# ChainSafe/Spectre

Hardware: AMD Instinct MI355X
Metric: BN254 G1 MSM n=2^20 throughput (higher is better)
Workload: dtype u256; 1 GPU; msm_g1_2pow20; n=1048576, seed=42, parallelism=shard1:window, pipeline_depth=3, scalars=canonical

## Files before the change

spectre_amd/csrc/ff.hpp:

```cpp
#pragma once
#include <stdint.h>
#include <string.h>

#if defined(__HIPCC__) || defined(__HIP_DEVICE_COMPILE__)
#include <hip/hip_runtime.h>
#define FF_HD __host__ __device__ __forceinline__
#else
#define FF_HD inline
#endif

struct fp256 {
    uint32_t l[8];
};

struct FqP {
    static constexpr bool kAsmMul = true;
    static constexpr bool kChainAddSub = true;
    FF_HD static constexpr uint32_t mod(int i) {
        constexpr uint32_t M[8] = {0xd87cfd47u, 0x3c208c16u, 0x6871ca8du, 0x97816a91u,
                                   0x8181585du, 0xb85045b6u, 0xe131a029u, 0x30644e72u};
        return M[i];
    }
    FF_HD static constexpr uint32_t inv() { return 0xe4866389u; }
    FF_HD static constexpr uint32_t r2(int i) {
// ... 61 lines not shown
        o.l[i] = (uint32_t)d;
        brw = (d >> 32) & 1;
    }
    return (uint32_t)brw;
}
FF_HD uint32_t ff_add_raw(fp256& o, const fp256& a, const fp256& b) {
    uint64_t c = 0;
    for (int i = 0; i < 8; i++) {
        c += (uint64_t)a.l[i] + b.l[i];
        o.l[i] = (uint32_t)c;
        c >>= 32;
    }
    return (uint32_t)c;
}
FF_HD uint32_t ff_adc_(uint32_t a, uint32_t b, uint32_t& carry) {
#if defined(__has_builtin) && __has_builtin(__builtin_addc)
    unsigned out;
    const uint32_t r = __builtin_addc(a, b, carry, &out);
    carry = out;
    return r;
#else
    const uint64_t s = (uint64_t)a + b + carry;
    carry = (uint32_t)(s >> 32);
    return (uint32_t)s;
#endif
}
FF_HD uint32_t ff_sbb_(uint32_t a, uint32_t b, uint32_t& borrow) {
#if defined(__has_builtin) && __has_builtin(__builtin_subc)
    unsigned out;
    const uint32_t r = __builtin_subc(a, b, borrow, &out);
    borrow = out;
    return r;
#else
    const uint64_t d = (uint64_t)a - b - borrow;
    borrow = (uint32_t)(d >> 32) & 1;
    return (uint32_t)d;
#endif
}
template <class C> FF_HD void ff_cond_sub_mod_chain_(fp256& o, uint32_t extra) {
    uint32_t d[8], brw = 0;
    for (int i = 0; i < 8; i++) d[i] = ff_sbb_(o.l[i], C::mod(i), brw);
    const bool keep = extra != 0 || brw == 0;
    for (int i = 0; i < 8; i++) o.l[i] = keep ? d[i] : o.l[i];
}
template <class C> FF_HD void ff_cond_sub_mod(fp256& o, uint32_t extra) {
    if constexpr (C::kChainAddSub) {
        ff_cond_sub_mod_chain_<C>(o, extra);
    } else if (extra || ff_geq_mod<C>(o)) {
        uint64_t brw = 0;
        for (int i = 0; i < 8; i++) {
            uint64_t d = (uint64_t)o.l[i] - C::mod(i) - brw;
            o.l[i] = (uint32_t)d;
            brw = (d >> 32) & 1;
        }
    }
}
template <class C> FF_HD void ff_add(fp256& o, const fp256& a, const fp256& b) {
    if constexpr (C::kChainAddSub) {
        uint32_t c = 0;
        for (int i = 0; i < 8; i++) o.l[i] = ff_adc_(a.l[i], b.l[i], c);
        ff_cond_sub_mod_chain_<C>(o, c);
    } else {
        uint32_t c = ff_add_raw(o, a, b);
        ff_cond_sub_mod<C>(o, c);
    }
}
template <class C> FF_HD void ff_sub(fp256& o, const fp256& a, const fp256& b) {
    if constexpr (C::kChainAddSub) {
        uint32_t brw = 0;
        for (int i = 0; i < 8; i++) o.l[i] = ff_sbb_(a.l[i], b.l[i], brw);
        const uint32_t mask = 0u - brw;
        uint32_t c = 0;
        for (int i = 0; i < 8; i++) o.l[i] = ff_adc_(o.l[i], C::mod(i) & mask, c);
    } else if (ff_sub_raw(o, a, b)) {
        uint64_t c = 0;
        for (int i = 0; i < 8; i++) {
            c += (uint64_t)o.l[i] + C::mod(i);
            o.l[i] = (uint32_t)c;
            c >>= 32;
        }
    }
}
template <class C> FF_HD void ff_neg(fp256& o, const fp256& a) {
    if (ff_is_zero(a)) { o = a; return; }
    fp256 m;
    for (int i = 0; i < 8; i++) m.l[i] = C::mod(i);
    ff_sub_raw(o, m, a);
}

template <class C> FF_HD void ff_mul_cios(fp256& o, const fp256& a, const fp256& b) {
    uint32_t t[10];
    for (int i = 0; i < 10; i++) t[i] = 0;
    for (int i = 0; i < 8; i++) {
        uint64_t cc = 0;
        const uint32_t ai = a.l[i];
        for (int j = 0; j < 8; j++) {
            uint64_t x = (uint64_t)ai * b.l[j] + t[j] + (uint32_t)cc;
            t[j] = (uint32_t)x;
            cc = x >> 32;
        }
        uint64_t x = (uint64_t)t[8] + (uint32_t)cc;
        t[8] = (uint32_t)x;
        t[9] = (uint32_t)(x >> 32);
        const uint32_t m = t[0] * C::inv();
        uint64_t x2 = (uint64_t)m * C::mod(0) + t[0];
        cc = x2 >> 32;
        for (int j = 1; j < 8; j++) {
            x2 = (uint64_t)m * C::mod(j) + t[j] + (uint32_t)cc;
            t[j - 1] = (uint32_t)x2;
            cc = x2 >> 32;
        }
        x2 = (uint64_t)t[8] + (uint32_t)cc;
        t[7] = (uint32_t)x2;
        t[8] = t[9] + (uint32_t)(x2 >> 32);
    }
    for (int i = 0; i < 8; i++) o.l[i] = t[i];
    ff_cond_sub_mod<C>(o, t[8]);
}
#if defined(__HIP_DEVICE_COMPILE__) && !defined(SPECTRE_NO_ASM_MUL)
#define FF_HAVE_ASM_MUL 1
#endif

#if defined(FF_HAVE_ASM_MUL)
__device__ __forceinline__ void ff_mad64_(uint64_t& acc, uint32_t& ovf,
                                          uint32_t a, uint32_t b) {
    uint64_t c;
    asm volatile("v_mad_u64_u32 %0, %2, %3, %4, %0\n\t"
                 "v_addc_co_u32 %1, %2, 0, %1, %2"
                 : "+v"(acc), "+v"(ovf), "=s"(c)
                 : "v"(a), "v"(b));
}
__device__ __forceinline__ void ff_mad64_s_(uint64_t& acc, uint32_t& ovf,
                                            uint32_t a, uint32_t b_uniform) {
    uint64_t c;
    asm volatile("v_mad_u64_u32 %0, %2, %3, %4, %0\n\t"
                 "v_addc_co_u32 %1, %2, 0, %1, %2"
                 : "+v"(acc), "+v"(ovf), "=s"(c)
                 : "v"(a), "s"(b_uniform));
}
template <class C, int K>
__device__ __forceinline__ void detail_ff_low_cols(uint64_t& acc,
                                                   uint32_t& ovf,
                                                   const uint32_t* a,
                                                   const uint32_t* b,
                                                   uint32_t* m) {
    if constexpr (K < 8) {
#pragma unroll
        for (int i = 0; i <= K; i++) ff_mad64_(acc, ovf, a[i], b[K - i]);
#pragma unroll
        for (int i = 0; i < K; i++) ff_mad64_s_(acc, ovf, m[i], C::mod(K - i));
        m[K] = (uint32_t)acc * C::inv();
        ff_mad64_s_(acc, ovf, m[K], C::mod(0));
        acc = (acc >> 32) | ((uint64_t)ovf << 32);
        ovf = 0;
        detail_ff_low_cols<C, K + 1>(acc, ovf, a, b, m);
    }
}
template <class C, int K>
__device__ __forceinline__ void detail_ff_high_cols(uint64_t& acc,
                                                    uint32_t& ovf,
                                                    const uint32_t* a,
                                                    const uint32_t* b,
                                                    const uint32_t* m,
                                                    uint32_t* out) {
    if constexpr (K < 15) {
#pragma unroll
// ... 6 lines not shown
        detail_ff_high_cols<C, K + 1>(acc, ovf, a, b, m, out);
    }
}
template <class C>
__device__ __forceinline__ void ff_mul_cols(fp256& o, const fp256& A,
                                            const fp256& B) {
    uint32_t m[8];
    uint64_t acc = 0;
    uint32_t ovf = 0;
    detail_ff_low_cols<C, 0>(acc, ovf, A.l, B.l, m);
    detail_ff_high_cols<C, 8>(acc, ovf, A.l, B.l, m, o.l);
    o.l[7] = (uint32_t)acc;
    ff_cond_sub_mod<C>(o, (uint32_t)(acc >> 32));
}

template <int K>
__device__ __forceinline__ void detail_ff_sqr_col(uint64_t& acc, uint32_t& ovf,
                                                  const uint32_t* a,
                                                  const uint32_t* adj,
                                                  const uint32_t* dbl) {
#pragma unroll
    for (int i = K < 8 ? 0 : K - 7; 2 * i + 1 < K; i++)
        ff_mad64_(acc, ovf, a[i], dbl[K - i]);
    if constexpr (K % 2) ff_mad64_(acc, ovf, a[K / 2], adj[K / 2 + 1]);
    else ff_mad64_(acc, ovf, a[K / 2], a[K / 2]);
}
template <class C, int K>
__device__ __forceinline__ void detail_ff_sqr_low_cols(uint64_t& acc,
                                                       uint32_t& ovf,
                                                       const uint32_t* a,
                                                       const uint32_t* adj,
                                                       const uint32_t* dbl,
                                                       uint32_t* m) {
    if constexpr (K < 8) {
        detail_ff_sqr_col<K>(acc, ovf, a, adj, dbl);
#pragma unroll
        for (int i = 0; i < K; i++) ff_mad64_s_(acc, ovf, m[i], C::mod(K - i));
        m[K] = (uint32_t)acc * C::inv();
        ff_mad64_s_(acc, ovf, m[K], C::mod(0));
        acc = (acc >> 32) | ((uint64_t)ovf << 32);
        ovf = 0;
        detail_ff_sqr_low_cols<C, K + 1>(acc, ovf, a, adj, dbl, m);
    }
}
template <class C, int K>
__device__ __forceinline__ void detail_ff_sqr_high_cols(uint64_t& acc,
                                                        uint32_t& ovf,
                                                        const uint32_t* a,
                                                        const uint32_t* adj,
                                                        const uint32_t* dbl,
                                                        const uint32_t* m,
                                                        uint32_t* out) {
    if constexpr (K < 15) {
        detail_ff_sqr_col<K>(acc, ovf, a, adj, dbl);
#pragma unroll
        for (int i = K - 7; i < 8; i++) ff_mad64_s_(acc, ovf, m[i], C::mod(K - i));
        out[K - 8] = (uint32_t)acc;
        acc = (acc >> 32) | ((uint64_t)ovf << 32);
        ovf = 0;
        detail_ff_sqr_high_cols<C, K + 1>(acc, ovf, a, adj, dbl, m, out);
    }
}
template <class C>
__device__ __forceinline__ void ff_sqr_cols(fp256& o, const fp256& A) {
    static_assert(C::mod(7) < 0x80000000u,
                  "the doubled limbs drop bit 255: reduced elements must be "
                  "below 2^255");
    uint32_t a[8], adj[8], dbl[8], m[8];
#pragma unroll
    for (int i = 0; i < 8; i++) a[i] = A.l[i];
    adj[0] = dbl[0] = 0;
#pragma unroll
    for (int j = 1; j < 8; j++) {
        adj[j] = a[j] << 1;
        dbl[j] = (a[j] << 1) | (a[j - 1] >> 31);
    }
    uint64_t acc = 0;
    uint32_t ovf = 0;
    detail_ff_sqr_low_cols<C, 0>(acc, ovf, a, adj, dbl, m);
    detail_ff_sqr_high_cols<C, 8>(acc, ovf, a, adj, dbl, m, o.l);
    o.l[7] = (uint32_t)acc;
    ff_cond_sub_mod<C>(o, (uint32_t)(acc >> 32));
}
#endif

template <class C> FF_HD void ff_mul(fp256& o, const fp256& a, const fp256& b) {
#if defined(FF_HAVE_ASM_MUL)
    if constexpr (C::kAsmMul) {
        ff_mul_cols<C>(o, a, b);
        return;
    }
#endif
    ff_mul_cios<C>(o, a, b);
}

template <class C> FF_HD void ff_sqr(fp256& o, const fp256& a) {
#if defined(FF_HAVE_ASM_MUL)
    if constexpr (C::kAsmMul) {
        ff_sqr_cols<C>(o, a);
        return;
    }
#endif
    ff_mul<C>(o, a, a);
}

template <class C> FF_HD void ff_to_mont(fp256& o, const fp256& a_canon) {
    fp256 r2;
    for (int i = 0; i < 8; i++) r2.l[i] = C::r2(i);
    ff_mul<C>(o, a_canon, r2);
}
template <class C> FF_HD void ff_from_mont(fp256& o, const fp256& a) {
    fp256 one;
    ff_set_zero(one);
    one.l[0] = 1;
    ff_mul<C>(o, a, one);
}

template <class C> FF_HD void ff_pow_u32(fp256& o, const fp256& a, uint32_t e) {
    fp256 acc, base = a;
    ff_set_one<C>(acc);
    while (e) {
        if (e & 1) ff_mul<C>(acc, acc, base);
        e >>= 1;
        if (e) ff_sqr<C>(base, base);
    }
    o = acc;
}
template <class C> FF_HD void ff_inv(fp256& o, const fp256& a) {
    static_assert(C::mod(0) >= 2u, "m - 2 must not borrow out of the low word");
    fp256 acc, base = a;
    ff_set_one<C>(acc);
#pragma unroll 1
    for (uint32_t w = 0; w < 8; w++) {
        uint32_t bits = C::mod(0) - 2u;
#pragma unroll
        for (uint32_t i = 1; i < 8; i++) bits = w == i ? C::mod(i) : bits;
#pragma unroll 1
        for (uint32_t b = 0; b < 32; b++) {
            if ((bits >> b) & 1) ff_mul<C>(acc, acc, base);
            ff_sqr<C>(base, base);
        }
    }
    o = acc;
}

FF_HD void ff_from_bytes(fp256& o, const uint8_t* b) { memcpy(o.l, b, 32); }
FF_HD void ff_to_bytes(uint8_t* b, const fp256& a) { memcpy(b, a.l, 32); }

using Fq = FqP;
using Fr = FrP;

#if defined(__HIPCC__) || defined(__HIP_DEVICE_COMPILE__)
__device__ __forceinline__ void lds_split_ld(const uint4* lds4, uint32_t lo,
                                             uint32_t dist, fp256& o) {
    uint4 l = lds4[lo], h = lds4[dist + lo];
    memcpy(&o.l[0], &l, 16);
    memcpy(&o.l[4], &h, 16);
}
__device__ __forceinline__ void lds_split_st(uint4* lds4, uint32_t lo,
                                             uint32_t dist, const fp256& v) {
    uint4 l, h;
    memcpy(&l, &v.l[0], 16);
    memcpy(&h, &v.l[4], 16);
    lds4[lo] = l;
    lds4[dist + lo] = h;
}
#endif
```

spectre_amd/csrc/g1.hpp:

```cpp
#pragma once
#include "ff.hpp"

struct g1_affine {
    fp256 x, y;
};
struct g1_jac {
    fp256 X, Y, Z;
};

FF_HD bool g1a_is_inf(const g1_affine& p) { return ff_is_zero(p.x) && ff_is_zero(p.y); }
FF_HD void g1j_set_inf(g1_jac& p) {
    ff_set_one<Fq>(p.X);
    ff_set_one<Fq>(p.Y);
    ff_set_zero(p.Z);
}
FF_HD bool g1j_is_inf(const g1_jac& p) { return ff_is_zero(p.Z); }
FF_HD void g1j_from_affine(g1_jac& o, const g1_affine& p) {
    if (g1a_is_inf(p)) { g1j_set_inf(o); return; }
    o.X = p.x;
    o.Y = p.y;
    ff_set_one<Fq>(o.Z);
}

FF_HD void g1j_dbl_ip(g1_jac& p) {
    if (g1j_is_inf(p)) return;
    fp256 A, B, C, D, E, F;
    ff_sqr<Fq>(A, p.X);
    ff_sqr<Fq>(B, p.Y);
    ff_sqr<Fq>(C, B);
    ff_add<Fq>(D, p.X, B);
    ff_sqr<Fq>(D, D);
    ff_sub<Fq>(D, D, A);
    ff_sub<Fq>(D, D, C);
    ff_add<Fq>(D, D, D);
    ff_add<Fq>(E, A, A);
    ff_add<Fq>(E, E, A);
    ff_sqr<Fq>(F, E);
    ff_mul<Fq>(p.Z, p.Y, p.Z);
    ff_add<Fq>(p.Z, p.Z, p.Z);
    ff_sub<Fq>(p.X, F, D);
    ff_sub<Fq>(p.X, p.X, D);
    ff_sub<Fq>(D, D, p.X);
    ff_mul<Fq>(D, E, D);
    ff_add<Fq>(C, C, C);
    ff_add<Fq>(C, C, C);
    ff_add<Fq>(C, C, C);
    ff_sub<Fq>(p.Y, D, C);
}

FF_HD void g1j_madd_ip(g1_jac& p, const g1_affine& q) {
    if (g1a_is_inf(q)) return;
    if (g1j_is_inf(p)) { g1j_from_affine(p, q); return; }
    fp256 Z1Z1, U2, S2, H, HH, I, J, rr, V;
    ff_sqr<Fq>(Z1Z1, p.Z);
    ff_mul<Fq>(U2, q.x, Z1Z1);
    ff_mul<Fq>(S2, q.y, p.Z);
    ff_mul<Fq>(S2, S2, Z1Z1);
    ff_sub<Fq>(H, U2, p.X);
    ff_sub<Fq>(rr, S2, p.Y);
    if (ff_is_zero(H)) {
        if (ff_is_zero(rr)) { g1j_dbl_ip(p); return; }
        g1j_set_inf(p);
        return;
    }
    ff_add<Fq>(rr, rr, rr);
    ff_sqr<Fq>(HH, H);
    ff_add<Fq>(I, HH, HH);
    ff_add<Fq>(I, I, I);
    ff_mul<Fq>(J, H, I);
    ff_mul<Fq>(V, p.X, I);
    ff_add<Fq>(p.Z, p.Z, H);
    ff_sqr<Fq>(p.Z, p.Z);
    ff_sub<Fq>(p.Z, p.Z, Z1Z1);
    ff_sub<Fq>(p.Z, p.Z, HH);
    ff_sqr<Fq>(H, rr);
    ff_sub<Fq>(H, H, J);
    ff_sub<Fq>(H, H, V);
    ff_sub<Fq>(H, H, V);
    ff_sub<Fq>(V, V, H);
    ff_mul<Fq>(V, rr, V);
    ff_mul<Fq>(J, p.Y, J);
    ff_add<Fq>(J, J, J);
    ff_sub<Fq>(p.Y, V, J);
    p.X = H;
}

FF_HD void g1j_add_ip(g1_jac& p, const g1_jac& q) {
    if (g1j_is_inf(q)) return;
    if (g1j_is_inf(p)) { p = q; return; }
    fp256 Z1Z1, Z2Z2, U1, U2, S1, S2, H, I, J, rr, V;
    ff_sqr<Fq>(Z1Z1, p.Z);
    ff_sqr<Fq>(Z2Z2, q.Z);
    ff_mul<Fq>(U1, p.X, Z2Z2);
    ff_mul<Fq>(U2, q.X, Z1Z1);
    ff_mul<Fq>(S1, p.Y, q.Z);
    ff_mul<Fq>(S1, S1, Z2Z2);
    ff_mul<Fq>(S2, q.Y, p.Z);
    ff_mul<Fq>(S2, S2, Z1Z1);
    ff_sub<Fq>(H, U2, U1);
    ff_sub<Fq>(rr, S2, S1);
    if (ff_is_zero(H)) {
        if (ff_is_zero(rr)) { g1j_dbl_ip(p); return; }
        g1j_set_inf(p);
        return;
    }
    ff_add<Fq>(rr, rr, rr);
    ff_add<Fq>(I, H, H);
    ff_sqr<Fq>(I, I);
    ff_mul<Fq>(J, H, I);
    ff_mul<Fq>(V, U1, I);
    ff_add<Fq>(p.Z, p.Z, q.Z);
    ff_sqr<Fq>(p.Z, p.Z);
    ff_sub<Fq>(p.Z, p.Z, Z1Z1);
    ff_sub<Fq>(p.Z, p.Z, Z2Z2);
    ff_mul<Fq>(p.Z, p.Z, H);
    ff_sqr<Fq>(H, rr);
    ff_sub<Fq>(H, H, J);
    ff_sub<Fq>(H, H, V);
    ff_sub<Fq>(H, H, V);
    ff_sub<Fq>(V, V, H);
    ff_mul<Fq>(V, rr, V);
    ff_mul<Fq>(J, S1, J);
    ff_add<Fq>(J, J, J);
    ff_sub<Fq>(p.Y, V, J);
    p.X = H;
}


FF_HD void g1j_to_affine(g1_affine& o, const g1_jac& p) {
    if (g1j_is_inf(p)) {
        ff_set_zero(o.x);
        ff_set_zero(o.y);
        return;
    }
    fp256 zi, zi2, zi3;
    ff_inv<Fq>(zi, p.Z);
    ff_sqr<Fq>(zi2, zi);
    ff_mul<Fq>(zi3, zi2, zi);
    ff_mul<Fq>(o.x, p.X, zi2);
    ff_mul<Fq>(o.y, p.Y, zi3);
}
```

spectre_amd/csrc/internal.hpp:

```cpp
#pragma once
#include <hip/hip_runtime.h>
#include "spectre_gpu.h"
#include "ff.hpp"
#include "g1.hpp"
#include "powtab.hpp"
#include <array>
#include <map>
#include <mutex>
#include <string>
#include <vector>

#define MSM_WBITS 16
#define MSM_NWIN 16
#define MSM_BPW (1u << (MSM_WBITS - 1))
#ifndef MSM_CHUNK
#define MSM_CHUNK SPECTRE_MSM_TAIL_CHUNK
#endif
#define MSM_CPW (MSM_BPW / MSM_CHUNK)
#define MSM_LO SPECTRE_MSM_TAIL_LO
#define MSM_HI (MSM_CPW / MSM_LO)
static_assert(MSM_CPW % MSM_LO == 0, "chunks per window: a multiple of MSM_LO");
static_assert((MSM_CHUNK & (MSM_CHUNK - 1)) == 0 && (MSM_LO & (MSM_LO - 1)) == 0,
              "the host fold multiplies by doubling");
#define MSM_ACC_E_MIN 8
#define MSM_ACC_E_MAX 64
#define MSM_ACC_TARGET_BLOCKS 2

void set_err(const char* fmt, ...);

#define HIP_TRY(x)                                                        \
    do {                                                                  \
        hipError_t _e = (x);                                              \
        if (_e != hipSuccess) {                                           \
            set_err("%s:%d %s: %s", __FILE__, __LINE__, #x,               \
                    hipGetErrorString(_e));                               \
            return -2;                                                    \
        }                                                                 \
    } while (0)

#define RC_TRY(x)                                                         \
    do {                                                                  \
        int _rc = (x);                                                    \
        if (_rc) return _rc;                                              \
    } while (0)

template <typename T, bool kPinned = false>
struct DevBuf {
    T* ptr = nullptr;
    size_t cap = 0;
    int reserve(size_t n) {
        if (cap >= n) return 0;
        release();
        void* p = nullptr;
        if (kPinned) HIP_TRY(hipHostMalloc(&p, n * sizeof(T)));
        else HIP_TRY(hipMalloc(&p, n * sizeof(T)));
        ptr = (T*)p;
        cap = n;
        return 0;
    }
    void release() {
        if (ptr) (void)(kPinned ? hipHostFree(ptr) : hipFree(ptr));
        ptr = nullptr;
        cap = 0;
    }
};
template <typename T>
using PinnedBuf = DevBuf<T, true>;
template <typename... B>
void release_all(B&... b) {
    (b.release(), ...);
}

struct NttPlan {
    uint32_t npass = 0;
    uint32_t k[3] = {};
    DevBuf<fp256> tw[3];
    DevBuf<fp256> twB;
    PowTable omega = {};
    void release() { release_all(tw[0], tw[1], tw[2], twB); }
};

#define MSM_SLOTS 3
struct MsmSlot {
    hipStream_t stream = nullptr;
    DevBuf<uint32_t> d_keys_in, d_keys_out, d_vals_in, d_vals_out;
    DevBuf<uint8_t> d_sort_tmp;
    DevBuf<uint32_t> d_firstK, d_lastK;
    DevBuf<g1_jac> d_firstP, d_lastP;
    DevBuf<uint32_t> d_offsets;
    DevBuf<g1_jac> d_buckets;
    DevBuf<g1_jac> d_red;
    PinnedBuf<g1_jac> h_wins;
    g1_jac* pending_dst = nullptr;
    uint32_t pending_n = 0;
    void release(hipStream_t shared) {
        release_all(d_keys_in, d_keys_out, d_vals_in, d_vals_out, d_sort_tmp,
                    d_firstK, d_lastK, d_firstP, d_lastP, d_offsets,
                    d_buckets, d_red, h_wins);
        if (stream && stream != shared) (void)hipStreamDestroy(stream);
        stream = nullptr;
    }
};

struct DeviceState {
    int device_id = 0;
    hipStream_t stream = nullptr;
    MsmSlot slots[MSM_SLOTS];
    int next_slot = 0;
    int num_cus = 0;
    int acc_resident_blocks = 0;
    DevBuf<uint8_t> d_scalars;
    DevBuf<g1_affine> d_bases;
    std::map<std::array<uint64_t, 3>, DevBuf<g1_affine>> bases_cache;
    DevBuf<fp256> d_ntt_io;
    PinnedBuf<uint8_t> h_stage[2];
    hipEvent_t stage_ev[2] = {nullptr, nullptr};
    DevBuf<uint8_t> d_call;
    PinnedBuf<uint8_t> h_call;
    std::map<std::array<uint8_t, 40>, NttPlan> plans;
    void release() {
        for (auto& sl : slots) sl.release(stream);
        release_all(d_scalars, d_bases, d_ntt_io, h_stage[0], h_stage[1],
                    d_call, h_call);
        for (auto& kv : bases_cache) kv.second.release();
        bases_cache.clear();
        for (auto& kv : plans) kv.second.release();
        plans.clear();
        for (auto& e : stage_ev) {
            if (e) (void)hipEventDestroy(e);
            e = nullptr;
        }
        if (stream) (void)hipStreamDestroy(stream);
        stream = nullptr;
    }
};

#define CALL_PINNED_BYTES \
    (SPECTRE_OPEN_MAX_POLYS * SPECTRE_POLY_EVAL_MAX_POINTS * 32u)
inline int call_finish(DeviceState& ds, void* dst = nullptr,
                       const void* d_src = nullptr, size_t bytes = 0) {
    if (dst) {
        RC_TRY(ds.h_call.reserve(CALL_PINNED_BYTES));
        HIP_TRY(hipMemcpyAsync(ds.h_call.ptr, d_src, bytes,
                               hipMemcpyDeviceToHost, ds.stream));
    }
    HIP_TRY(hipStreamSynchronize(ds.stream));
    HIP_TRY(hipGetLastError());
    if (dst) memcpy(dst, ds.h_call.ptr, bytes);
    return 0;
}

struct spectre_gpu_ctx {
    std::vector<DeviceState> devs;
    std::recursive_mutex mu;
    uint32_t msm_acc_entries = 0;
    uint32_t fr_scan_tile = 0;
    bool ntt_force3 = false;
};

struct MsmCall {
    const g1_affine* d_bases;
    const uint8_t* d_scalars;
    uint32_t nbatch;
    uint64_t n;
    uint32_t flags;
    uint32_t w_lo, w_cnt;
};

int msm_device(spectre_gpu_ctx* ctx, int dev, const MsmCall& call,
               g1_jac* winsums_host, double* stage_ms, bool sync, int slot);

uint32_t msm_acc_auto_entries(uint64_t entries, uint32_t cus,
                              uint32_t resident_blocks);

int msm_slot_drain(spectre_gpu_ctx* ctx, int dev, int slot);

void msm_fold_window(const g1_jac& p0, const g1_jac& p1, const g1_jac& p2,
                     g1_jac& out);

int fr_gate_eval_device(spectre_gpu_ctx* ctx, int dev,
                        const fp256* const* cols, uint32_t ncols,
// ... 56 lines not shown
```

spectre_amd/csrc/msm.hip:

```cpp
#include "internal.hpp"
#include <hipcub/hipcub.hpp>

#define THREADS 256
#define PT_KERNEL __global__ __launch_bounds__(THREADS, 2)
#ifndef MSM_ACC_THREADS
#define MSM_ACC_THREADS 256
#endif
#define ACC_KERNEL __global__ __launch_bounds__(MSM_ACC_THREADS, 2)

__global__ void k_msm_digits(const uint8_t* __restrict__ scalars, uint64_t n,
                             uint32_t nbatch, int canonical, uint32_t w_lo,
                             uint32_t w_cnt,
                             uint32_t* __restrict__ keys,
                             uint32_t* __restrict__ vals) {
    uint64_t i = (uint64_t)blockIdx.x * blockDim.x + threadIdx.x;
    if (i >= n) return;
    const uint32_t nb_local = w_cnt * MSM_BPW;
    const uint32_t skip_key = nbatch * nb_local;
    for (uint32_t b = 0; b < nbatch; b++) {
        fp256 s;
        ff_from_bytes(s, scalars + 32 * (b * n + i));
        if (!canonical) ff_from_mont<Fr>(s, s);
        uint32_t carry = 0;
        for (int w = 0; w < MSM_NWIN; w++) {
            const uint32_t bit0 = (uint32_t)w * MSM_WBITS;
            const uint32_t li = bit0 >> 5, sh = bit0 & 31;
            uint64_t pair = (uint64_t)s.l[li];
            if (li < 7) pair |= (uint64_t)s.l[li + 1] << 32;
            uint32_t d =
                ((uint32_t)(pair >> sh) & ((1u << MSM_WBITS) - 1)) + carry;
            const uint32_t half = 1u << (MSM_WBITS - 1);
            const uint32_t full = 1u << MSM_WBITS;
            uint32_t key, val = (uint32_t)i;
            if (d == 0) {
                carry = 0;
                key = skip_key;
            } else if (d <= half) {
                carry = 0;
                key = b * nb_local + ((uint32_t)w - w_lo) * MSM_BPW + (d - 1);
            } else if (d == full) {
                carry = 1;
                key = skip_key;
            } else {
                carry = 1;
                key = b * nb_local + ((uint32_t)w - w_lo) * MSM_BPW +
                      (full - d - 1);
                val |= 0x80000000u;
            }
            if ((uint32_t)w < w_lo || (uint32_t)w >= w_lo + w_cnt) continue;
            const uint64_t slot =
                ((uint64_t)b * w_cnt + ((uint32_t)w - w_lo)) * n + i;
            keys[slot] = key;
            vals[slot] = val;
        }
    }
}

__global__ void k_bucket_offsets(const uint32_t* __restrict__ keys,
                                 uint64_t nent, uint32_t nb_total,
                                 uint32_t* __restrict__ off) {
    uint32_t b = blockIdx.x * blockDim.x + threadIdx.x;
    if (b > nb_total) return;
    uint64_t lo = 0, hi = nent;
    while (lo < hi) {
        uint64_t mid = (lo + hi) >> 1;
        if (keys[mid] < b) lo = mid + 1;
        else hi = mid;
    }
    off[b] = (uint32_t)lo;
}

#define ACC_WAVES (MSM_ACC_THREADS / 64)
__device__ __forceinline__ void glds16(const void* src, uint4* wave_dst) {
    __builtin_amdgcn_global_load_lds(
        (const __attribute__((address_space(1))) void*)src,
        (__attribute__((address_space(3))) void*)wave_dst, 16, 0, 0);
}
__device__ __forceinline__ void glds_landed() {
    asm volatile("s_waitcnt vmcnt(0)" ::: "memory");
}
__device__ __forceinline__ void lds_reads_done() {
    asm volatile("s_waitcnt lgkmcnt(0)" ::: "memory");
}

ACC_KERNEL void k_bucket_acc(const uint32_t* __restrict__ off,
                            const uint32_t* __restrict__ keys,
                            const uint32_t* __restrict__ vals,
                            const g1_affine* __restrict__ bases,
                            uint32_t nb_total, uint32_t E,
                            g1_jac* __restrict__ buckets,
                            uint32_t* __restrict__ firstK,
                            g1_jac* __restrict__ firstP,
                            uint32_t* __restrict__ lastK,
                            g1_jac* __restrict__ lastP) {
    __shared__ uint4 stage[ACC_WAVES][8][64];
    const uint32_t ent = off[nb_total];
    const uint32_t t = blockIdx.x * blockDim.x + threadIdx.x;
    const uint64_t lo = (uint64_t)t * E;
    if (lo >= ent) return;
    const uint32_t cnt = ent - lo < E ? (uint32_t)(ent - lo) : E;
    const uint4* kq = (const uint4*)(keys + lo);
    const uint4* vq = (const uint4*)(vals + lo);
    const uint32_t lane = threadIdx.x & 63;
    uint4(*st)[64] = stage[threadIdx.x >> 6];
    glds16(kq, st[4]);
    glds16(vq, st[6]);
    glds_landed();
    uint32_t k = st[4][lane].x;
    {
        const uint4* src = (const uint4*)(bases + (st[6][lane].x & 0x7fffffffu));
        for (int c = 0; c < 4; c++) glds16(src + c, st[c]);
    }
    g1_jac acc;
    g1j_set_inf(acc);
    bool first = true;
    for (uint32_t i = 0; i < cnt; i++) {
        glds_landed();
        const uint32_t q = 4 + ((i >> 2) & 1);
        const uint32_t kj = ((const uint32_t*)&st[q][lane])[i & 3];
        const uint32_t v = ((const uint32_t*)&st[q + 2][lane])[i & 3];
        g1_affine p;
        {
            const uint4 x0 = st[0][lane], x1 = st[1][lane];
            const uint4 y0 = st[2][lane], y1 = st[3][lane];
            p.x.l[0] = x0.x; p.x.l[1] = x0.y; p.x.l[2] = x0.z; p.x.l[3] = x0.w;
            p.x.l[4] = x1.x; p.x.l[5] = x1.y; p.x.l[6] = x1.z; p.x.l[7] = x1.w;
            p.y.l[0] = y0.x; p.y.l[1] = y0.y; p.y.l[2] = y0.z; p.y.l[3] = y0.w;
            p.y.l[4] = y1.x; p.y.l[5] = y1.y; p.y.l[6] = y1.z; p.y.l[7] = y1.w;
        }
        if (i + 1 < cnt) {
            const uint32_t qn = 6 + (((i + 1) >> 2) & 1);
            const uint32_t vn = ((const uint32_t*)&st[qn][lane])[(i + 1) & 3];
            lds_reads_done();
            if ((i & 3) == 0 && i + 4 < cnt) {
                const uint32_t qf = 4 + (((i >> 2) + 1) & 1);
                glds16(kq + (i >> 2) + 1, st[qf]);
                glds16(vq + (i >> 2) + 1, st[qf + 2]);
            }
            const uint4* src = (const uint4*)(bases + (vn & 0x7fffffffu));
            for (int c = 0; c < 4; c++) glds16(src + c, st[c]);
        }
        if (kj != k) {
            if (first) {
                firstK[t] = k;
                firstP[t] = acc;
                first = false;
            } else {
                buckets[k] = acc;
            }
            g1j_set_inf(acc);
            k = kj;
        }
        if (v & 0x80000000u) ff_neg<Fq>(p.y, p.y);
        g1j_madd_ip(acc, p);
    }
    if (first) {
        firstK[t] = k;
        firstP[t] = acc;
        lastK[t] = 0xffffffffu;
    } else {
        lastK[t] = k;
        lastP[t] = acc;
    }
}

ACC_KERNEL void k_bucket_fix(const uint32_t* __restrict__ off,
                            const uint32_t* __restrict__ firstK,
                            const g1_jac* __restrict__ firstP,
                            const uint32_t* __restrict__ lastK,
                            const g1_jac* __restrict__ lastP,
                            uint32_t nb_total, uint32_t E,
                            g1_jac* __restrict__ buckets) {
    uint32_t b = blockIdx.x * blockDim.x + threadIdx.x;
    if (b >= nb_total) return;
    uint32_t s = off[b], e = off[b + 1];
    if (s == e) {
        g1j_set_inf(buckets[b]);
        return;
    }
    uint32_t ts = s / E, te = (e - 1) / E;
    const uint32_t ent = off[nb_total];
    if (ts == te && (s % E) && (e % E) && e != ent)
        return;
    g1_jac acc;
    g1j_set_inf(acc);
    for (uint32_t t = ts; t <= te; t++) {
        if (firstK[t] == b) g1j_add_ip(acc, firstP[t]);
        if (lastK[t] == b) g1j_add_ip(acc, lastP[t]);
    }
    buckets[b] = acc;
}

PT_KERNEL void k_window_chunks(const g1_jac* __restrict__ buckets,
                               uint32_t total_chunks,
                               g1_jac* __restrict__ outW,
                               g1_jac* __restrict__ outT) {
    uint32_t t = blockIdx.x * blockDim.x + threadIdx.x;
    if (t >= total_chunks) return;
    const g1_jac* B = buckets + (uint64_t)t * MSM_CHUNK;
    g1_jac accT, accW;
    g1j_set_inf(accT);
    g1j_set_inf(accW);
    for (int j = MSM_CHUNK - 1; j >= 0; j--) {
        g1j_add_ip(accT, B[j]);
        g1j_add_ip(accW, accT);
    }
    outW[t] = accW;
    outT[t] = accT;
}

#ifndef WSUM_THREADS
#define WSUM_THREADS 512
#endif
static_assert(MSM_CPW % WSUM_THREADS == 0, "role 0 shares");
static_assert(WSUM_THREADS % MSM_LO == 0 && MSM_HI % (WSUM_THREADS / MSM_LO) == 0,
              "column shares");
static_assert(MSM_HI <= WSUM_THREADS && WSUM_THREADS % MSM_HI == 0 &&
              MSM_LO % (WSUM_THREADS / MSM_HI) == 0, "row shares");
__global__ __launch_bounds__(WSUM_THREADS, 2) void k_window_tail(
    const g1_jac* __restrict__ inW, const g1_jac* __restrict__ inT,
    g1_jac* __restrict__ out) {
    __shared__ g1_jac lds[WSUM_THREADS / 2];
    const uint32_t w = blockIdx.x / 3, role = blockIdx.x % 3;
    const uint32_t t = threadIdx.x;
    const uint32_t M = role == 0 ? 0 : role == 1 ? MSM_LO : MSM_HI;
    const g1_jac* src;
    uint32_t stride, cnt;
    if (role == 0) {
        src = inW + (uint64_t)w * MSM_CPW + t;
        stride = WSUM_THREADS;
        cnt = MSM_CPW / WSUM_THREADS;
    } else if (role == 1) {
        cnt = MSM_HI / (WSUM_THREADS / MSM_LO);
        src = inT + (uint64_t)w * MSM_CPW + (t / MSM_LO) * cnt * MSM_LO +
              t % MSM_LO;
        stride = MSM_LO;
    } else {
        cnt = MSM_LO / (WSUM_THREADS / MSM_HI);
        src = inT + (uint64_t)w * MSM_CPW + (t % MSM_HI) * MSM_LO +
              (t / MSM_HI) * cnt;
        stride = 1;
    }
    g1_jac acc;
    g1j_set_inf(acc);
    for (uint32_t j = 0; j < cnt; j++) g1j_add_ip(acc, src[(uint64_t)j * stride]);
    for (uint32_t k = WSUM_THREADS / 2; k >= 1; k >>= 1) {
        if (2 * k == M && t < M) {
            if (t == 0) g1j_set_inf(acc);
            if (!g1j_is_inf(acc)) {
                g1_jac r;
                g1j_set_inf(r);
                for (uint32_t bit = M >> 1; bit; bit >>= 1) {
                    g1j_dbl_ip(r);
                    if (t & bit) g1j_add_ip(r, acc);
                }
                acc = r;
            }
        }
        if (t >= k && t < 2 * k) lds[t - k] = acc;
        __syncthreads();
        if (t < k) g1j_add_ip(acc, lds[t]);
        __syncthreads();
    }
    if (t == 0) out[blockIdx.x] = acc;
}

uint32_t msm_acc_auto_entries(uint64_t entries, uint32_t cus,
                              uint32_t resident_blocks) {
    uint32_t per_cu = resident_blocks ? resident_blocks : 1;
    if (per_cu > MSM_ACC_TARGET_BLOCKS) per_cu = MSM_ACC_TARGET_BLOCKS;
    const uint64_t threads =
        (uint64_t)(cus ? cus : 1) * per_cu * MSM_ACC_THREADS;
    if (entries >= threads * MSM_ACC_E_MAX) return MSM_ACC_E_MAX;
    uint64_t e = (entries + threads - 1) / threads;
    e = (e + 3) & ~3ull;
    if (e < MSM_ACC_E_MIN) e = MSM_ACC_E_MIN;
    if (e > MSM_ACC_E_MAX) e = MSM_ACC_E_MAX;
    return (uint32_t)e;
}

static int ensure_acc_geometry(DeviceState& dstate) {
    if (dstate.acc_resident_blocks) return 0;
    int cus = 0, nb = 0;
    HIP_TRY(hipDeviceGetAttribute(&cus, hipDeviceAttributeMultiprocessorCount,
                                  dstate.device_id));
    HIP_TRY(hipOccupancyMaxActiveBlocksPerMultiprocessor(
        &nb, k_bucket_acc, MSM_ACC_THREADS, 0));
    dstate.num_cus = cus > 0 ? cus : 1;
    dstate.acc_resident_blocks = nb > 0 ? nb : 1;
    return 0;
}

static int ensure_msm_scratch(MsmSlot& ds, uint64_t ent, uint32_t nwin,
                              uint32_t acc_e) {
    const uint64_t nbt = (uint64_t)nwin * MSM_BPW;
    const uint64_t ent4 = (ent + 3) & ~3ull;
    for (auto* b : {&ds.d_keys_in, &ds.d_keys_out, &ds.d_vals_in,
                    &ds.d_vals_out})
        RC_TRY(b->reserve(ent4));
    const uint64_t nt = (ent + acc_e - 1) / acc_e;
    RC_TRY(ds.d_firstK.reserve(nt));
    RC_TRY(ds.d_lastK.reserve(nt));
    RC_TRY(ds.d_firstP.reserve(nt));
    RC_TRY(ds.d_lastP.reserve(nt));
    RC_TRY(ds.d_offsets.reserve(nbt + 1));
    RC_TRY(ds.d_buckets.reserve(nbt));
    RC_TRY(ds.d_red.reserve(2 * nbt / MSM_CHUNK + 3 * (uint64_t)nwin));
    size_t sort_need = 0;
    (void)hipcub::DeviceRadixSort::SortPairs(
        nullptr, sort_need, ds.d_keys_in.ptr, ds.d_keys_out.ptr,
        ds.d_vals_in.ptr, ds.d_vals_out.ptr, (int64_t)ent, 0, 32, ds.stream);
    return ds.d_sort_tmp.reserve(sort_need);
}

static int end_bit_for(uint64_t max_key) {
    int b = 0;
    while ((1ull << b) <= max_key) b++;
    return b;
}

struct StageTimer {
    hipEvent_t ev[7] = {};
    hipStream_t st = nullptr;
    hipError_t err = hipSuccess;
    uint32_t ent_real = 0;
    bool on = false;
    ~StageTimer() {
        for (auto e : ev)
            if (e) (void)hipEventDestroy(e);
    }
    int start(hipStream_t s) {
        on = true;
        st = s;
        for (auto& e : ev) HIP_TRY(hipEventCreate(&e));
        return 0;
    }
    void stamp(int i) {
        if (on && err == hipSuccess) err = hipEventRecord(ev[i], st);
    }
    int read(double* stage_ms) {
        HIP_TRY(err);
        float ms;
        for (int i = 0; i < 6; i++) {
            HIP_TRY(hipEventElapsedTime(&ms, ev[i], ev[i + 1]));
            stage_ms[i] = ms;
        }
        HIP_TRY(hipEventElapsedTime(&ms, ev[0], ev[6]));
        stage_ms[6] = ms;
        stage_ms[7] = (double)ent_real;
        return 0;
    }
};

static int msm_acquire_slot(DeviceState& dstate, const MsmCall& c, int slot,
                            MsmSlot** out) {
    HIP_TRY(hipSetDevice(dstate.device_id));
    if (slot < 0 || slot >= MSM_SLOTS) {
        set_err("msm: slot %d out of range", slot);
        return -3;
    }
    MsmSlot& ds = dstate.slots[slot];
    if (ds.pending_dst) {
        set_err("msm: slot %d already has a call in flight", slot);
        return -3;
    }
    if (!ds.stream) {
        if (slot == 0) ds.stream = dstate.stream;
        else HIP_TRY(hipStreamCreate(&ds.stream));
    }
    if (c.nbatch == 0 || c.nbatch > SPECTRE_MSM_MAX_BATCH) {
        set_err("msm: nbatch %u out of range [1,%d]", c.nbatch,
                SPECTRE_MSM_MAX_BATCH);
        return -3;
    }
    if (c.w_lo >= MSM_NWIN || c.w_cnt == 0 || c.w_lo + c.w_cnt > MSM_NWIN) {
        set_err("msm: window range [%u, %u+%u) out of [0,%d)", c.w_lo, c.w_lo,
                c.w_cnt, MSM_NWIN);
        return -3;
    }
    if ((uint64_t)c.nbatch * c.w_cnt * c.n >= (1ull << 32)) {
        set_err("msm: nbatch*%u*n = %llu exceeds 2^32 sort-entry limit "
                "(split the batch or shard the MSM)", c.w_cnt,
                (unsigned long long)((uint64_t)c.nbatch * c.w_cnt * c.n));
        return -3;
    }
    *out = &ds;
    return 0;
}

static int msm_enqueue(spectre_gpu_ctx* ctx, DeviceState& dstate, MsmSlot& ds,
                       const MsmCall& c, g1_jac* winsums_host,
                       StageTimer& timer) {
    const uint32_t nw = c.nbatch * c.w_cnt;
    const uint64_t ent = (uint64_t)nw * c.n;
    RC_TRY(ensure_acc_geometry(dstate));
    const uint32_t acc_e =
        ctx->msm_acc_entries
            ? ctx->msm_acc_entries
            : msm_acc_auto_entries(ent, (uint32_t)dstate.num_cus,
                                   (uint32_t)dstate.acc_resident_blocks);
    RC_TRY(ensure_msm_scratch(ds, ent, nw, acc_e));
    RC_TRY(ds.h_wins.reserve(3 * (size_t)nw));
    const uint32_t nbt = nw * MSM_BPW;
    const int canonical = (c.flags & SPECTRE_SCALARS_CANONICAL) ? 1 : 0;
    hipStream_t st = ds.stream;

    timer.stamp(0);
    uint32_t blocks = (uint32_t)((c.n + THREADS - 1) / THREADS);
    hipLaunchKernelGGL(k_msm_digits, dim3(blocks), dim3(THREADS), 0, st,
                       c.d_scalars, c.n, c.nbatch, canonical, c.w_lo, c.w_cnt,
                       ds.d_keys_in.ptr, ds.d_vals_in.ptr);
    timer.stamp(1);
    size_t tmp = ds.d_sort_tmp.cap;
    (void)hipcub::DeviceRadixSort::SortPairs(
        ds.d_sort_tmp.ptr, tmp, ds.d_keys_in.ptr, ds.d_keys_out.ptr,
        ds.d_vals_in.ptr, ds.d_vals_out.ptr, (int64_t)ent, 0,
        end_bit_for(nbt), st);
    timer.stamp(2);
    hipLaunchKernelGGL(k_bucket_offsets,
                       dim3((nbt + 1 + THREADS - 1) / THREADS), dim3(THREADS),
                       0, st, ds.d_keys_out.ptr, ent, nbt, ds.d_offsets.ptr);
    timer.stamp(3);
    const uint32_t nt_acc = (uint32_t)((ent + acc_e - 1) / acc_e);
    hipLaunchKernelGGL(k_bucket_acc,
                       dim3((nt_acc + MSM_ACC_THREADS - 1) / MSM_ACC_THREADS),
                       dim3(MSM_ACC_THREADS), 0, st, ds.d_offsets.ptr,
                       ds.d_keys_out.ptr, ds.d_vals_out.ptr, c.d_bases, nbt,
                       acc_e, ds.d_buckets.ptr, ds.d_firstK.ptr,
                       ds.d_firstP.ptr, ds.d_lastK.ptr, ds.d_lastP.ptr);
    hipLaunchKernelGGL(k_bucket_fix,
                       dim3((nbt + MSM_ACC_THREADS - 1) / MSM_ACC_THREADS),
                       dim3(MSM_ACC_THREADS), 0, st, ds.d_offsets.ptr,
                       ds.d_firstK.ptr, ds.d_firstP.ptr, ds.d_lastK.ptr,
                       ds.d_lastP.ptr, nbt, acc_e, ds.d_buckets.ptr);
    timer.stamp(4);
    const uint32_t nchunks = nbt / MSM_CHUNK;
    g1_jac* redW = ds.d_red.ptr;
    g1_jac* redT = redW + nchunks;
    g1_jac* redP = redT + nchunks;
    hipLaunchKernelGGL(k_window_chunks,
                       dim3((nchunks + THREADS - 1) / THREADS), dim3(THREADS),
                       0, st, ds.d_buckets.ptr, nchunks, redW, redT);
    timer.stamp(5);
    hipLaunchKernelGGL(k_window_tail, dim3(3 * nw), dim3(WSUM_THREADS), 0, st,
                       redW, redT, redP);
    timer.stamp(6);
    HIP_TRY(hipMemcpyAsync(ds.h_wins.ptr, redP,
                           3 * (size_t)nw * sizeof(g1_jac),
                           hipMemcpyDeviceToHost, st));
    if (timer.on)
        HIP_TRY(hipMemcpyAsync(&timer.ent_real, ds.d_offsets.ptr + nbt, 4,
                               hipMemcpyDeviceToHost, st));
    HIP_TRY(hipGetLastError());
    ds.pending_dst = winsums_host;
    ds.pending_n = nw;
    return 0;
}

void msm_fold_window(const g1_jac& p0, const g1_jac& p1, const g1_jac& p2,
                     g1_jac& out) {
    g1_jac acc = p2;
    for (uint32_t m = MSM_LO; m > 1; m >>= 1) g1j_dbl_ip(acc);
    g1j_add_ip(acc, p1);
    for (uint32_t m = MSM_CHUNK; m > 1; m >>= 1) g1j_dbl_ip(acc);
    g1j_add_ip(acc, p0);
    out = acc;
}

int msm_slot_drain(spectre_gpu_ctx* ctx, int dev, int slot) {
    DeviceState& dstate = ctx->devs[dev];
    if (slot < 0 || slot >= MSM_SLOTS) {
        set_err("slot_drain: slot %d out of range", slot);
        return -1;
    }
    MsmSlot& sl = dstate.slots[slot];
    g1_jac* const dst = sl.pending_dst;
    const uint32_t nw = sl.pending_n;
    sl.pending_dst = nullptr;
    sl.pending_n = 0;
    HIP_TRY(hipSetDevice(dstate.device_id));
    if (sl.stream) HIP_TRY(hipStreamSynchronize(sl.stream));
    HIP_TRY(hipGetLastError());
    if (dst) {
        const g1_jac* p = sl.h_wins.ptr;
        for (uint32_t w = 0; w < nw; w++, p += 3) {
            g1_jac sum;
            msm_fold_window(p[0], p[1], p[2], sum);
            memcpy((uint8_t*)dst + w * sizeof sum, &sum, sizeof sum);
        }
    }
    return 0;
}

int msm_device(spectre_gpu_ctx* ctx, int dev, const MsmCall& call,
               g1_jac* winsums_host, double* stage_ms, bool sync, int slot) {
    DeviceState& dstate = ctx->devs[dev];
    MsmSlot* sl = nullptr;
    RC_TRY(msm_acquire_slot(dstate, call, slot, &sl));
    if (call.n == 0) {
        for (uint32_t w = 0; w < call.nbatch * call.w_cnt; w++)
            g1j_set_inf(winsums_host[w]);
        return 0;
    }
    StageTimer timer;
    if (stage_ms) RC_TRY(timer.start(sl->stream));
    RC_TRY(msm_enqueue(ctx, dstate, *sl, call, winsums_host, timer));
    if (!sync && !stage_ms) return 0;
    RC_TRY(msm_slot_drain(ctx, dev, slot));
    return stage_ms ? timer.read(stage_ms) : 0;
}
```

Baseline: 444.9 MSM(2^20)/s.

## Switch bucket accumulation and reduction to XYZZ coordinates with fused dot-product reduction

Replaces Jacobian coordinates with extended XYZZ coordinates in the bucket accumulation, fix-up, chunk and window-tail kernels. Mixed additions in XYZZ need fewer field multiplies than Jacobian madd. It also adds a fused a*b+c*d Montgomery product (dot2), which shares one reduction across two products, and a branchless chained negation. In exchange each point grows from three to four field elements, adding memory traffic and register pressure, and a conversion back to Jacobian is needed at the window output.

After: 518.1 MSM(2^20)/s, median of 6. 16.5% higher.

```diff
diff --git a/spectre_amd/csrc/ff.hpp b/spectre_amd/csrc/ff.hpp
--- a/spectre_amd/csrc/ff.hpp
+++ b/spectre_amd/csrc/ff.hpp
@@ -167,6 +167,12 @@
     }
 }
 template <class C> FF_HD void ff_neg(fp256& o, const fp256& a) {
+    if constexpr (C::kChainAddSub) {
+        fp256 z;
+        ff_set_zero(z);
+        ff_sub<C>(o, z, a);
+        return;
+    }
     if (ff_is_zero(a)) { o = a; return; }
     fp256 m;
     for (int i = 0; i < 8; i++) m.l[i] = C::mod(i);
@@ -339,6 +345,58 @@
     o.l[7] = (uint32_t)acc;
     ff_cond_sub_mod<C>(o, (uint32_t)(acc >> 32));
 }
+
+template <class C, int K>
+__device__ __forceinline__ void detail_ff_dot2_low_cols(
+    uint64_t& acc, uint32_t& ovf, const uint32_t* a, const uint32_t* b,
+    const uint32_t* c, const uint32_t* d, uint32_t* m) {
+    if constexpr (K < 8) {
+#pragma unroll
+        for (int i = 0; i <= K; i++) {
+            ff_mad64_(acc, ovf, a[i], b[K - i]);
+            ff_mad64_(acc, ovf, c[i], d[K - i]);
+        }
+#pragma unroll
+        for (int i = 0; i < K; i++) ff_mad64_s_(acc, ovf, m[i], C::mod(K - i));
+        m[K] = (uint32_t)acc * C::inv();
+        ff_mad64_s_(acc, ovf, m[K], C::mod(0));
+        acc = (acc >> 32) | ((uint64_t)ovf << 32);
+        ovf = 0;
+        detail_ff_dot2_low_cols<C, K + 1>(acc, ovf, a, b, c, d, m);
+    }
+}
+template <class C, int K>
+__device__ __forceinline__ void detail_ff_dot2_high_cols(
+    uint64_t& acc, uint32_t& ovf, const uint32_t* a, const uint32_t* b,
+    const uint32_t* c, const uint32_t* d, const uint32_t* m, uint32_t* out) {
+    if constexpr (K < 15) {
+#pragma unroll
+        for (int i = K - 7; i < 8; i++) {
+            ff_mad64_(acc, ovf, a[i], b[K - i]);
+            ff_mad64_(acc, ovf, c[i], d[K - i]);
+        }
+#pragma unroll
+        for (int i = K - 7; i < 8; i++) ff_mad64_s_(acc, ovf, m[i], C::mod(K - i));
+        out[K - 8] = (uint32_t)acc;
+        acc = (acc >> 32) | ((uint64_t)ovf << 32);
+        ovf = 0;
+        detail_ff_dot2_high_cols<C, K + 1>(acc, ovf, a, b, c, d, m, out);
+    }
+}
+template <class C>
+__device__ __forceinline__ void ff_dot2_cols(fp256& o, const fp256& A,
+                                             const fp256& B, const fp256& Cc,
+                                             const fp256& D) {
+    static_assert(C::mod(7) < 0x80000000u,
+                  "one trial subtract after a*b + c*d needs 2m <= 2^256");
+    uint32_t m[8];
+    uint64_t acc = 0;
+    uint32_t ovf = 0;
+    detail_ff_dot2_low_cols<C, 0>(acc, ovf, A.l, B.l, Cc.l, D.l, m);
+    detail_ff_dot2_high_cols<C, 8>(acc, ovf, A.l, B.l, Cc.l, D.l, m, o.l);
+    o.l[7] = (uint32_t)acc;
+    ff_cond_sub_mod<C>(o, (uint32_t)(acc >> 32));
+}
 #endif
 
 template <class C> FF_HD void ff_mul(fp256& o, const fp256& a, const fp256& b) {
@@ -359,6 +417,21 @@
     }
 #endif
     ff_mul<C>(o, a, a);
+}
+
+template <class C>
+FF_HD void ff_dot2(fp256& o, const fp256& a, const fp256& b, const fp256& c,
+                   const fp256& d) {
+#if defined(FF_HAVE_ASM_MUL)
+    if constexpr (C::kAsmMul) {
+        ff_dot2_cols<C>(o, a, b, c, d);
+        return;
+    }
+#endif
+    fp256 t;
+    ff_mul<C>(t, a, b);
+    ff_mul<C>(o, c, d);
+    ff_add<C>(o, t, o);
 }
 
 template <class C> FF_HD void ff_to_mont(fp256& o, const fp256& a_canon) {
diff --git a/spectre_amd/csrc/g1.hpp b/spectre_amd/csrc/g1.hpp
--- a/spectre_amd/csrc/g1.hpp
+++ b/spectre_amd/csrc/g1.hpp
@@ -78,10 +78,9 @@
     ff_sub<Fq>(H, H, V);
     ff_sub<Fq>(H, H, V);
     ff_sub<Fq>(V, V, H);
-    ff_mul<Fq>(V, rr, V);
-    ff_mul<Fq>(J, p.Y, J);
-    ff_add<Fq>(J, J, J);
-    ff_sub<Fq>(p.Y, V, J);
+    ff_add<Fq>(p.Y, p.Y, p.Y);
+    ff_neg<Fq>(p.Y, p.Y);
+    ff_dot2<Fq>(p.Y, rr, V, p.Y, J);
     p.X = H;
 }
 
@@ -119,13 +118,108 @@
     ff_sub<Fq>(H, H, V);
     ff_sub<Fq>(H, H, V);
     ff_sub<Fq>(V, V, H);
-    ff_mul<Fq>(V, rr, V);
-    ff_mul<Fq>(J, S1, J);
-    ff_add<Fq>(J, J, J);
-    ff_sub<Fq>(p.Y, V, J);
+    ff_add<Fq>(S1, S1, S1);
+    ff_neg<Fq>(S1, S1);
+    ff_dot2<Fq>(p.Y, rr, V, S1, J);
     p.X = H;
 }
 
+struct g1_xyzz {
+    fp256 X, Y, ZZ, ZZZ;
+};
+FF_HD void g1x_set_inf(g1_xyzz& p) {
+    ff_set_one<Fq>(p.X);
+    ff_set_one<Fq>(p.Y);
+    ff_set_zero(p.ZZ);
+    ff_set_zero(p.ZZZ);
+}
+FF_HD bool g1x_is_inf(const g1_xyzz& p) { return ff_is_zero(p.ZZ); }
+FF_HD void g1x_from_affine(g1_xyzz& o, const g1_affine& p) {
+    if (g1a_is_inf(p)) { g1x_set_inf(o); return; }
+    o.X = p.x;
+    o.Y = p.y;
+    ff_set_one<Fq>(o.ZZ);
+    ff_set_one<Fq>(o.ZZZ);
+}
+
+FF_HD void g1x_dbl_ip(g1_xyzz& p) {
+    if (g1x_is_inf(p)) return;
+    fp256 U, V, W, S, M;
+    ff_add<Fq>(U, p.Y, p.Y);
+    ff_sqr<Fq>(V, U);
+    ff_mul<Fq>(W, U, V);
+    ff_mul<Fq>(S, p.X, V);
+    ff_sqr<Fq>(M, p.X);
+    ff_add<Fq>(U, M, M);
+    ff_add<Fq>(M, U, M);
+    ff_mul<Fq>(p.ZZ, V, p.ZZ);
+    ff_mul<Fq>(p.ZZZ, W, p.ZZZ);
+    ff_sqr<Fq>(p.X, M);
+    ff_sub<Fq>(p.X, p.X, S);
+    ff_sub<Fq>(p.X, p.X, S);
+    ff_sub<Fq>(S, S, p.X);
+    ff_neg<Fq>(p.Y, p.Y);
+    ff_dot2<Fq>(p.Y, M, S, p.Y, W);
+}
+
+FF_HD bool g1x_add_core_(g1_xyzz& p, const fp256& U1, fp256& S1, fp256& U2,
+                         fp256& S2, fp256& PP, fp256& PPP) {
+    ff_sub<Fq>(U2, U2, U1);
+    ff_sub<Fq>(S2, S2, S1);
+    if (ff_is_zero(U2)) {
+        if (ff_is_zero(S2)) g1x_dbl_ip(p);
+        else g1x_set_inf(p);
+        return false;
+    }
+    fp256 Q;
+    ff_sqr<Fq>(PP, U2);
+    ff_mul<Fq>(PPP, U2, PP);
+    ff_mul<Fq>(Q, U1, PP);
+    ff_sqr<Fq>(p.X, S2);
+    ff_sub<Fq>(p.X, p.X, PPP);
+    ff_sub<Fq>(p.X, p.X, Q);
+    ff_sub<Fq>(p.X, p.X, Q);
+    ff_sub<Fq>(Q, Q, p.X);
+    ff_neg<Fq>(S1, S1);
+    ff_dot2<Fq>(p.Y, S2, Q, S1, PPP);
+    return true;
+}
+
+FF_HD void g1x_madd_ip(g1_xyzz& p, const g1_affine& q) {
+    if (g1a_is_inf(q)) return;
+    if (g1x_is_inf(p)) { g1x_from_affine(p, q); return; }
+    fp256 U1 = p.X, S1 = p.Y, U2, S2, PP, PPP;
+    ff_mul<Fq>(U2, q.x, p.ZZ);
+    ff_mul<Fq>(S2, q.y, p.ZZZ);
+    if (!g1x_add_core_(p, U1, S1, U2, S2, PP, PPP)) return;
+    ff_mul<Fq>(p.ZZ, p.ZZ, PP);
+    ff_mul<Fq>(p.ZZZ, p.ZZZ, PPP);
+}
+
+FF_HD void g1x_add_ip(g1_xyzz& p, const g1_xyzz& q) {
+    if (g1x_is_inf(q)) return;
+    if (g1x_is_inf(p)) { p = q; return; }
+    fp256 U1, S1, U2, S2, PP, PPP;
+    ff_mul<Fq>(U1, p.X, q.ZZ);
+    ff_mul<Fq>(S1, p.Y, q.ZZZ);
+    ff_mul<Fq>(U2, q.X, p.ZZ);
+    ff_mul<Fq>(S2, q.Y, p.ZZZ);
+    if (!g1x_add_core_(p, U1, S1, U2, S2, PP, PPP)) return;
+    ff_mul<Fq>(p.ZZ, p.ZZ, q.ZZ);
+    ff_mul<Fq>(p.ZZ, p.ZZ, PP);
+    ff_mul<Fq>(p.ZZZ, p.ZZZ, q.ZZZ);
+    ff_mul<Fq>(p.ZZZ, p.ZZZ, PPP);
+}
+
+FF_HD void g1x_to_jac(g1_jac& o, const g1_xyzz& p) {
+    if (g1x_is_inf(p)) { g1j_set_inf(o); return; }
+    fp256 t;
+    ff_sqr<Fq>(t, p.ZZ);
+    ff_mul<Fq>(o.X, p.X, t);
+    ff_sqr<Fq>(t, p.ZZZ);
+    ff_mul<Fq>(o.Y, p.Y, t);
+    o.Z = p.ZZZ;
+}
 
 FF_HD void g1j_to_affine(g1_affine& o, const g1_jac& p) {
     if (g1j_is_inf(p)) {
diff --git a/spectre_amd/csrc/internal.hpp b/spectre_amd/csrc/internal.hpp
--- a/spectre_amd/csrc/internal.hpp
+++ b/spectre_amd/csrc/internal.hpp
@@ -86,17 +86,18 @@
     DevBuf<uint32_t> d_keys_in, d_keys_out, d_vals_in, d_vals_out;
     DevBuf<uint8_t> d_sort_tmp;
     DevBuf<uint32_t> d_firstK, d_lastK;
-    DevBuf<g1_jac> d_firstP, d_lastP;
+    DevBuf<g1_xyzz> d_firstP, d_lastP;
     DevBuf<uint32_t> d_offsets;
-    DevBuf<g1_jac> d_buckets;
-    DevBuf<g1_jac> d_red;
+    DevBuf<g1_xyzz> d_buckets;
+    DevBuf<g1_xyzz> d_red;
+    DevBuf<g1_jac> d_part;
     PinnedBuf<g1_jac> h_wins;
     g1_jac* pending_dst = nullptr;
     uint32_t pending_n = 0;
     void release(hipStream_t shared) {
         release_all(d_keys_in, d_keys_out, d_vals_in, d_vals_out, d_sort_tmp,
                     d_firstK, d_lastK, d_firstP, d_lastP, d_offsets,
-                    d_buckets, d_red, h_wins);
+                    d_buckets, d_red, d_part, h_wins);
         if (stream && stream != shared) (void)hipStreamDestroy(stream);
         stream = nullptr;
     }
diff --git a/spectre_amd/csrc/msm.hip b/spectre_amd/csrc/msm.hip
--- a/spectre_amd/csrc/msm.hip
+++ b/spectre_amd/csrc/msm.hip
@@ -88,11 +88,11 @@
                             const uint32_t* __restrict__ vals,
                             const g1_affine* __restrict__ bases,
                             uint32_t nb_total, uint32_t E,
-                            g1_jac* __restrict__ buckets,
+                            g1_xyzz* __restrict__ buckets,
                             uint32_t* __restrict__ firstK,
-                            g1_jac* __restrict__ firstP,
+                            g1_xyzz* __restrict__ firstP,
                             uint32_t* __restrict__ lastK,
-                            g1_jac* __restrict__ lastP) {
+                            g1_xyzz* __restrict__ lastP) {
     __shared__ uint4 stage[ACC_WAVES][8][64];
     const uint32_t ent = off[nb_total];
     const uint32_t t = blockIdx.x * blockDim.x + threadIdx.x;
@@ -111,8 +111,8 @@
         const uint4* src = (const uint4*)(bases + (st[6][lane].x & 0x7fffffffu));
         for (int c = 0; c < 4; c++) glds16(src + c, st[c]);
     }
-    g1_jac acc;
-    g1j_set_inf(acc);
+    g1_xyzz acc;
+    g1x_set_inf(acc);
     bool first = true;
     for (uint32_t i = 0; i < cnt; i++) {
         glds_landed();
@@ -148,11 +148,11 @@
             } else {
                 buckets[k] = acc;
             }
-            g1j_set_inf(acc);
+            g1x_set_inf(acc);
             k = kj;
         }
         if (v & 0x80000000u) ff_neg<Fq>(p.y, p.y);
-        g1j_madd_ip(acc, p);
+        g1x_madd_ip(acc, p);
     }
     if (first) {
         firstK[t] = k;
@@ -164,46 +164,59 @@
     }
 }
 
+__device__ __forceinline__ g1_xyzz pt_load(const g1_xyzz* src) {
+    static_assert(sizeof(g1_xyzz) == 8 * sizeof(uint4), "four 32-byte elements");
+    uint4 q[8];
+#pragma unroll
+    for (int i = 0; i < 8; i++) q[i] = ((const uint4*)src)[i];
+#pragma unroll
+    for (int i = 0; i < 8; i++)
+        asm volatile("" : "+v"(q[i].x), "+v"(q[i].y), "+v"(q[i].z), "+v"(q[i].w));
+    g1_xyzz v;
+    memcpy(&v, q, sizeof v);
+    return v;
+}
+
 ACC_KERNEL void k_bucket_fix(const uint32_t* __restrict__ off,
                             const uint32_t* __restrict__ firstK,
-                            const g1_jac* __restrict__ firstP,
+                            const g1_xyzz* __restrict__ firstP,
                             const uint32_t* __restrict__ lastK,
-                            const g1_jac* __restrict__ lastP,
+                            const g1_xyzz* __restrict__ lastP,
                             uint32_t nb_total, uint32_t E,
-                            g1_jac* __restrict__ buckets) {
+                            g1_xyzz* __restrict__ buckets) {
     uint32_t b = blockIdx.x * blockDim.x + threadIdx.x;
     if (b >= nb_total) return;
     uint32_t s = off[b], e = off[b + 1];
     if (s == e) {
-        g1j_set_inf(buckets[b]);
+        g1x_set_inf(buckets[b]);
         return;
     }
     uint32_t ts = s / E, te = (e - 1) / E;
     const uint32_t ent = off[nb_total];
     if (ts == te && (s % E) && (e % E) && e != ent)
         return;
-    g1_jac acc;
-    g1j_set_inf(acc);
+    g1_xyzz acc;
+    g1x_set_inf(acc);
     for (uint32_t t = ts; t <= te; t++) {
-        if (firstK[t] == b) g1j_add_ip(acc, firstP[t]);
-        if (lastK[t] == b) g1j_add_ip(acc, lastP[t]);
+        if (firstK[t] == b) g1x_add_ip(acc, pt_load(firstP + t));
+        if (lastK[t] == b) g1x_add_ip(acc, pt_load(lastP + t));
     }
     buckets[b] = acc;
 }
 
-PT_KERNEL void k_window_chunks(const g1_jac* __restrict__ buckets,
+PT_KERNEL void k_window_chunks(const g1_xyzz* __restrict__ buckets,
                                uint32_t total_chunks,
-                               g1_jac* __restrict__ outW,
-                               g1_jac* __restrict__ outT) {
+                               g1_xyzz* __restrict__ outW,
+                               g1_xyzz* __restrict__ outT) {
     uint32_t t = blockIdx.x * blockDim.x + threadIdx.x;
     if (t >= total_chunks) return;
-    const g1_jac* B = buckets + (uint64_t)t * MSM_CHUNK;
-    g1_jac accT, accW;
-    g1j_set_inf(accT);
-    g1j_set_inf(accW);
+    const g1_xyzz* B = buckets + (uint64_t)t * MSM_CHUNK;
+    g1_xyzz accT, accW;
+    g1x_set_inf(accT);
+    g1x_set_inf(accW);
     for (int j = MSM_CHUNK - 1; j >= 0; j--) {
-        g1j_add_ip(accT, B[j]);
-        g1j_add_ip(accW, accT);
+        g1x_add_ip(accT, pt_load(B + j));
+        g1x_add_ip(accW, accT);
     }
     outW[t] = accW;
     outT[t] = accT;
@@ -218,13 +231,13 @@
 static_assert(MSM_HI <= WSUM_THREADS && WSUM_THREADS % MSM_HI == 0 &&
               MSM_LO % (WSUM_THREADS / MSM_HI) == 0, "row shares");
 __global__ __launch_bounds__(WSUM_THREADS, 2) void k_window_tail(
-    const g1_jac* __restrict__ inW, const g1_jac* __restrict__ inT,
+    const g1_xyzz* __restrict__ inW, const g1_xyzz* __restrict__ inT,
     g1_jac* __restrict__ out) {
-    __shared__ g1_jac lds[WSUM_THREADS / 2];
+    __shared__ __align__(16) g1_xyzz lds[WSUM_THREADS / 2];
     const uint32_t w = blockIdx.x / 3, role = blockIdx.x % 3;
     const uint32_t t = threadIdx.x;
     const uint32_t M = role == 0 ? 0 : role == 1 ? MSM_LO : MSM_HI;
-    const g1_jac* src;
+    const g1_xyzz* src;
     uint32_t stride, cnt;
     if (role == 0) {
         src = inW + (uint64_t)w * MSM_CPW + t;
@@ -241,28 +254,29 @@
               (t / MSM_HI) * cnt;
         stride = 1;
     }
-    g1_jac acc;
-    g1j_set_inf(acc);
-    for (uint32_t j = 0; j < cnt; j++) g1j_add_ip(acc, src[(uint64_t)j * stride]);
+    g1_xyzz acc;
+    g1x_set_inf(acc);
+    for (uint32_t j = 0; j < cnt; j++)
+        g1x_add_ip(acc, pt_load(src + (uint64_t)j * stride));
     for (uint32_t k = WSUM_THREADS / 2; k >= 1; k >>= 1) {
         if (2 * k == M && t < M) {
-            if (t == 0) g1j_set_inf(acc);
-            if (!g1j_is_inf(acc)) {
-                g1_jac r;
-                g1j_set_inf(r);
+            if (t == 0) g1x_set_inf(acc);
+            if (!g1x_is_inf(acc)) {
+                g1_xyzz r;
+                g1x_set_inf(r);
                 for (uint32_t bit = M >> 1; bit; bit >>= 1) {
-                    g1j_dbl_ip(r);
-                    if (t & bit) g1j_add_ip(r, acc);
+                    g1x_dbl_ip(r);
+                    if (t & bit) g1x_add_ip(r, acc);
                 }
                 acc = r;
             }
         }
         if (t >= k && t < 2 * k) lds[t - k] = acc;
         __syncthreads();
-        if (t < k) g1j_add_ip(acc, lds[t]);
+        if (t < k) g1x_add_ip(acc, pt_load(lds + t));
         __syncthreads();
     }
-    if (t == 0) out[blockIdx.x] = acc;
+    if (t == 0) g1x_to_jac(out[blockIdx.x], acc);
 }
 
 uint32_t msm_acc_auto_entries(uint64_t entries, uint32_t cus,
@@ -305,7 +319,8 @@
     RC_TRY(ds.d_lastP.reserve(nt));
     RC_TRY(ds.d_offsets.reserve(nbt + 1));
     RC_TRY(ds.d_buckets.reserve(nbt));
-    RC_TRY(ds.d_red.reserve(2 * nbt / MSM_CHUNK + 3 * (uint64_t)nwin));
+    RC_TRY(ds.d_red.reserve(2 * nbt / MSM_CHUNK));
+    RC_TRY(ds.d_part.reserve(3 * (uint64_t)nwin));
     size_t sort_need = 0;
     (void)hipcub::DeviceRadixSort::SortPairs(
         nullptr, sort_need, ds.d_keys_in.ptr, ds.d_keys_out.ptr,
@@ -435,9 +450,9 @@
                        ds.d_lastP.ptr, nbt, acc_e, ds.d_buckets.ptr);
     timer.stamp(4);
     const uint32_t nchunks = nbt / MSM_CHUNK;
-    g1_jac* redW = ds.d_red.ptr;
-    g1_jac* redT = redW + nchunks;
-    g1_jac* redP = redT + nchunks;
+    g1_xyzz* redW = ds.d_red.ptr;
+    g1_xyzz* redT = redW + nchunks;
+    g1_jac* redP = ds.d_part.ptr;
     hipLaunchKernelGGL(k_window_chunks,
                        dim3((nchunks + THREADS - 1) / THREADS), dim3(THREADS),
                        0, st, ds.d_buckets.ptr, nchunks, redW, redT);
```
